# darkAlert/sports-field-homography

Hardware: AMD Instinct MI355X
Metric: frames/sec at 640x360 batch=16 (1/2/4/8 GPU) + homography L1 vs ref (higher is better)
Workload: dtype f16x3->f32 (2-way fp16 split operands = 22 significand bits, 3 fp16 MFMA products, fp32 accumulate; end-to-end error at the level of an fp32 run, see DESIGN.md section 2); 1 GPU; predict(): UNet seg + ResNet34-STN + nearest warp, 640x360, batch 16/GPU, req_outputs=theta,warp_mask; global_batch=16, precision=f16x3, range_fallbacks=0, range_rescales=0, range_raises=0, parallelism=single GPU

## Files before the change

include/sfh_amd.h:

```cpp
#ifndef SFH_AMD_H
#define SFH_AMD_H

#include <stdint.h>

#ifdef __cplusplus
extern "C" {
#endif

#define SFH_OK 0
#define SFH_E_ARG (-1)
#define SFH_E_LAUNCH (-2)

#define SFH_TILE_8x32 0
#define SFH_TILE_16x16 1
#define SFH_TILE_32x8 2
#define SFH_TILE_8x16 3
#define SFH_TILE_16x8 4

#define SFH_FMT_F32 0
#define SFH_FMT_S3 1
#define SFH_FMT_H2 2
#define SFH_FMT_FH2 3
#define SFH_H2_ACT_EXP 2

// ... 36 lines not shown
  int32_t h2_exp_src, h2_exp_dst, h2_exp_res;
  uint32_t* h2_range;
  int32_t wg_couts;
  int32_t split_arith;
  int32_t ksplit;
  int64_t ksplit_stride;
  const float* acc_init;
  double* stats_partial;
  int32_t stats_rows;
  const float* bwd_z;
  const float* bwd_mi;
  const float* bwd_gamma;
  const float* bwd_beta;
  const float* up_wpacked;
  const float* up_scale;
} sfh_conv_desc;

const char* sfh_last_error(void);
int sfh_version(void);

int sfh_conv_fwd(const sfh_conv_desc* d, void* stream);

int sfh_conv_s3_fwd(const sfh_conv_desc* d, void* stream);
int64_t sfh_packed_s3_weight_bytes(int ksize, int c0, int c1, int cout_virtual);
int sfh_pack_s3_weights(const float* w, void* packed, int ksize, int c0, int c1, int cout_virtual,
                        int mode, int aux, void* stream);
int sfh_f32_to_s3(const float* src, void* dst, int64_t rows, int W, int cs, void* stream);
int sfh_s3_to_f32(const void* src, float* dst, int64_t rows, int W, int cs, void* stream);

int64_t sfh_packed_h2_weight_bytes(int ksize, int c0, int c1, int cout_virtual);
int sfh_pack_h2_weights(const float* w, void* packed, int ksize, int c0, int c1, int cout_virtual,
                        int mode, int aux, int wexp, void* stream);
int sfh_f32_to_h2(const float* src, void* dst, int64_t rows, int W, int cs, int act_exp, uint32_t* overflow,
                  uint32_t* range, void* stream);
int sfh_h2_to_f32(const void* src, float* dst, int64_t rows, int W, int cs, int act_exp, void* stream);

int sfh_conv_small_fwd(const sfh_conv_desc* d, void* stream);

int sfh_conv_upfused_fwd(const sfh_conv_desc* d, void* stream);

int sfh_conv3x3_c4_fwd(const sfh_conv_desc* d, void* stream);
int sfh_pack_c4_weights(const float* w, float* packed, int cin, int cout, void* stream);

int sfh_frame_to_h2(const float* src_nchw, float* dst_nhwc4, void* dst_fh2, int batch, int C, int H, int W, int act_exp,
                    uint32_t* overflow, uint32_t* range, void* stream);
int64_t sfh_packed_c4h2_weight_bytes(int cout);
// ... 203 lines not shown
```

sports-field-homography_amd/_lib.py:

```python
import ctypes as C
import os

_HERE = os.path.dirname(os.path.abspath(__file__))
LIB_PATH = os.environ.get("SFH_AMD_LIB") or os.path.join(_HERE, "libsfh_amd.so")

TILE_8x32, TILE_16x16, TILE_32x8, TILE_8x16, TILE_16x8 = 0, 1, 2, 3, 4
OUT_NHWC, OUT_UPSCATTER2 = 0, 1
FMT_F32, FMT_S3, FMT_H2, FMT_FH2 = 0, 1, 2, 3
H2_ACT_EXP = 2
H2_LIMIT_BITS = 0x477FE000

_p = C.c_void_p
_i = C.c_int32


class ConvDesc(C.Structure):
    _fields_ = [
        ("src0", _p), ("c0", _i), ("cs0", _i), ("h0", _i), ("w0", _i), ("pool0", _i),
        ("src1", _p), ("c1", _i), ("cs1", _i), ("h1", _i), ("w1", _i), ("pad_top1", _i), ("pad_left1", _i),
        ("batch", _i), ("H", _i), ("W", _i), ("ksize", _i), ("stride", _i), ("tile", _i),
        ("wpacked", _p), ("scale", _p), ("shift", _p), ("cout", _i), ("relu", _i),
        ("residual", _p),
        ("dst", _p), ("dst_cs", _i), ("out_mode", _i),
        ("src_fmt", _i), ("dst_fmt", _i), ("dst_pool", _p), ("pool_cs", _i),
        ("residual_f32", _i), ("shift_border", _p), ("up_dst_h", _i), ("up_dst_w", _i),
        ("reverse_tiles", _i),
        ("head_w", _p), ("head_b", _p), ("head_nc", _i), ("head_skip_dst", _i),
        ("head_logits", _p), ("head_stn", _p), ("head_frame", _p),
        ("h2_overflow", _p), ("h2_exp_src", _i), ("h2_exp_dst", _i), ("h2_exp_res", _i), ("h2_range", _p),
        ("wg_couts", _i), ("split_arith", _i), ("ksplit", _i), ("ksplit_stride", C.c_int64), ("acc_init", _p),
        ("stats_partial", _p), ("stats_rows", _i),
        ("bwd_z", _p), ("bwd_mi", _p), ("bwd_gamma", _p), ("bwd_beta", _p),
        ("up_wpacked", _p), ("up_scale", _p),
    ]

    def __init__(self, *args, **kw):
        super().__init__(*args, **kw)
        if "h2_exp_src" not in kw:
            self.h2_exp_src = self.h2_exp_dst = self.h2_exp_res = H2_ACT_EXP


SIGNATURES = {
    "sfh_last_error": (C.c_char_p, []),
    "sfh_version": (C.c_int, []),
    "sfh_conv_fwd": (C.c_int, [C.POINTER(ConvDesc), _p]),
    "sfh_conv_s3_fwd": (C.c_int, [C.POINTER(ConvDesc), _p]),
    "sfh_packed_s3_weight_bytes": (C.c_int64, [C.c_int, C.c_int, C.c_int, C.c_int]),
    "sfh_pack_s3_weights": (C.c_int, [_p, _p, C.c_int, C.c_int, C.c_int, C.c_int, C.c_int, C.c_int, _p]),
    "sfh_f32_to_s3": (C.c_int, [_p, _p, C.c_int64, C.c_int, C.c_int, _p]),
    "sfh_s3_to_f32": (C.c_int, [_p, _p, C.c_int64, C.c_int, C.c_int, _p]),
    "sfh_packed_h2_weight_bytes": (C.c_int64, [C.c_int, C.c_int, C.c_int, C.c_int]),
    "sfh_pack_h2_weights": (C.c_int, [_p, _p, C.c_int, C.c_int, C.c_int, C.c_int, C.c_int, C.c_int, C.c_int, _p]),
    "sfh_f32_to_h2": (C.c_int, [_p, _p, C.c_int64, C.c_int, C.c_int, C.c_int, _p, _p, _p]),
    "sfh_h2_to_f32": (C.c_int, [_p, _p, C.c_int64, C.c_int, C.c_int, C.c_int, _p]),
    "sfh_conv3x3_c4_fwd": (C.c_int, [C.POINTER(ConvDesc), _p]),
    "sfh_pack_c4_weights": (C.c_int, [_p, _p, C.c_int, C.c_int, _p]),
    "sfh_frame_to_h2": (C.c_int, [_p, _p, _p, C.c_int, C.c_int, C.c_int, C.c_int, C.c_int, _p, _p, _p]),
    "sfh_packed_c4h2_weight_bytes": (C.c_int64, [C.c_int]),
    "sfh_pack_c4h2_weights": (C.c_int, [_p, _p, C.c_int, C.c_int, C.c_int, _p]),
    "sfh_conv3x3_c4h2_fwd": (C.c_int, [C.POINTER(ConvDesc), _p]),
    "sfh_conv_small_fwd": (C.c_int, [C.POINTER(ConvDesc), _p]),
    "sfh_conv_upfused_fwd": (C.c_int, [C.POINTER(ConvDesc), _p]),
    "sfh_packed_weight_floats": (C.c_int64, [C.c_int, C.c_int, C.c_int, C.c_int]),
    "sfh_pack_conv_weights": (C.c_int, [_p, _p, C.c_int, C.c_int, C.c_int, C.c_int, C.c_int, C.c_int, _p]),
    "sfh_space_to_depth2": (C.c_int, [_p, _p, C.c_int, C.c_int, C.c_int, C.c_int, _p]),
    "sfh_fold_bn": (C.c_int, [_p, _p, _p, _p, _p, C.c_float, C.c_int, C.c_int, _p, _p, _p]),
    "sfh_u8hwc_to_f32nchw": (C.c_int, [_p, _p, C.c_int, C.c_int, C.c_int, C.c_int, _p]),
    "sfh_u8hwc_area2_to_f32nchw": (C.c_int, [_p, _p, C.c_int, C.c_int, C.c_int, C.c_int, _p]),
    "sfh_u8hwc_areak_to_f32nchw": (C.c_int, [_p, _p, C.c_int, C.c_int, C.c_int, C.c_int, C.c_int, _p]),
# ... 120 lines not shown
```

sports-field-homography_amd/csrc/conv_s3.hip:

```cpp
#include <stdlib.h>

#include <type_traits>

#include "common.h"
#include "conv_epilogue.h"

typedef unsigned int u32x4 __attribute__((ext_vector_type(4)));
typedef unsigned int u32x2 __attribute__((ext_vector_type(2)));
typedef __bf16 bf16x8 __attribute__((ext_vector_type(8)));
typedef _Float16 f16x8 __attribute__((ext_vector_type(8)));

namespace {

constexpr unsigned kOOB = 0xFFFFFFF0u;

#ifndef SFH_STAGE_PRIO
#define SFH_STAGE_PRIO 0
#endif

template <int KS_, int STRIDE_, int SH_, int SW_, int TH_, int TW_, int NP_ = 3, int NWN_ = 2, int NWM_ = 2, bool STATS_ = false>
struct S3Cfg {
  static constexpr int KS = KS_, STRIDE = STRIDE_, NP = NP_, NWN = NWN_, NWM = NWM_;
  static constexpr bool STATS = STATS_;
  static constexpr int NT = 64 * NWM * NWN;
// ... 124 lines not shown
    }
  }
}

}

namespace {

#ifndef SFH_H2_WD
#define SFH_H2_WD 2
#endif
#ifndef SFH_H2_XD
#define SFH_H2_XD 2
#endif
#ifndef SFH_W128_NWM
#define SFH_W128_NWM 1
#endif
#ifndef SFH_W8_MIN_BLOCKS
#define SFH_W8_MIN_BLOCKS 384
#endif
#ifndef SFH_H2_WAVES_PER_SIMD
#define SFH_H2_WAVES_PER_SIMD 2
#endif
template <class C, bool DB>
__global__ __launch_bounds__(C::NT, (C::NP == 2 && !DB) ? SFH_H2_WAVES_PER_SIMD : 2) void conv_s3_kernel(const sfh_conv_desc d,
                                                                                                     const S3Geom g) {
  extern __shared__ __attribute__((aligned(16))) float smem_f[];
  u32x4* const lds = reinterpret_cast<u32x4*>(smem_f);
  typedef __attribute__((address_space(3))) void* lds_ptr_t;
  SFH_STAMP_INIT();
  SFH_CLOCK_BEGIN();

  const int tid = threadIdx.x;
  const int lane = tid & 63;
  const int wv = __builtin_amdgcn_readfirstlane(tid >> 6);
  const int wm = wv / C::NWN, wn = wv % C::NWN;
  const int lq = lane & 15, lg = lane >> 4;

  const int ksn = d.ksplit > 1 ? d.ksplit : 1;
  const int per_split = (int)(gridDim.x / (unsigned)ksn);
  const int ks = ksn > 1 ? (int)blockIdx.x / per_split : 0;
  const int bid = (int)blockIdx.x - ks * per_split;
  const int xcd = bid & 7, kk_ = bid >> 3;
  const int tpx = (g.ntiles + 7) >> 3;
  const int per = tpx * g.nb_group;
  const int gi = kk_ / per, rr = kk_ - gi * per;
  const int nb = gi * g.nb_group + rr % g.nb_group;
  const int tl = d.reverse_tiles ? tpx - 1 - rr / g.nb_group : rr / g.nb_group;
  const int tile = xcd * tpx + tl;
// ... 5 lines not shown
    r0 = ty * C::TH;
  } else {
    const int img = ty / g.tiles_y;
    r0 = (img << 16) | ((ty - img * g.tiles_y) * C::TH);
  }
  const int n0 = nb * C::NCO;

  const int nst0 = d.c0 / C::CKS;
  const int nst1 = d.src1 ? d.c1 / C::CKS : 0;
  const int nst = nst0 + nst1;
  const int st0 = ks * nst / ksn, st1 = (ks + 1) * nst / ksn;

  const __amdgpu_buffer_rsrc_t rs0 =
      __builtin_amdgcn_make_buffer_rsrc(const_cast<float*>(d.src0), 0, (int)g.bytes0, 0x00020000);
  const __amdgpu_buffer_rsrc_t rs1 = __builtin_amdgcn_make_buffer_rsrc(
      const_cast<float*>(d.src1 ? d.src1 : d.src0), 0, (int)(d.src1 ? g.bytes1 : 0u), 0x00020000);
  constexpr int NP = C::NP;
  constexpr unsigned WTAP = (unsigned)NP * 4u * 1024u;
  const unsigned wtotal = (unsigned)nst * C::NTAP * WTAP;
  const __amdgpu_buffer_rsrc_t rsw = __builtin_amdgcn_make_buffer_rsrc(
      const_cast<char*>(reinterpret_cast<const char*>(d.wpacked)) + (size_t)(nb * (C::NWN / 2) + (wn >> 1)) * wtotal, 0,
      (int)wtotal, 0x00020000);
  const unsigned wvoff = lane * 16u + (unsigned)(2 * (wn & 1)) * 1024u;

  int pad_y = C::PAD, pad_x = C::PAD;
  if (C::KS == 2) {
    const int qd = n0 / (d.cout >> 2);
    pad_y = 1 - (qd >> 1);
    pad_x = 1 - (qd & 1);
  }
  unsigned hoff[C::NSL];
  s3_halo_offsets<C>(d, g, 0, tid, r0, x0, pad_y, pad_x, hoff);

  auto dma_piece = [&](int st, int b, int i) {
    u32x4* const hb = lds + b * C::BUF;
    const bool first = st < nst0;
    constexpr unsigned SB = 64u * (unsigned)NP;
    const unsigned cb = first ? (unsigned)st * (SB * (unsigned)d.w0) : (unsigned)(st - nst0) * (SB * (unsigned)d.w1);
    __builtin_amdgcn_raw_ptr_buffer_load_lds(first ? rs0 : rs1, (lds_ptr_t)(hb + wv * 64 + C::NT * i), 16,
                                             (int)hoff[i], (int)cb, 0, 0);
  };
  auto dma_stage = [&](int st, int b) {
#pragma unroll
    for (int i = 0; i < C::NSL; ++i) dma_piece(st, b, i);
  };

  auto load_w = [&](u32x4 (&w)[NP][2], unsigned soff) {
#pragma unroll
    for (int p = 0; p < NP; ++p)
#pragma unroll
      for (int ni = 0; ni < 2; ++ni)
        w[p][ni] = __builtin_amdgcn_raw_buffer_load_b128(rsw, (int)(wvoff + ni * 1024u), (int)(soff + p * 4096u), 0);
  };

  const int pixbase0 = lg * C::HPIXP +
                       ((wm * C::MT_M / C::SUBX) * C::SH + lq / C::SW) * C::STRIDE * C::HW +
                       (lq % C::SW) * C::STRIDE;
  static_assert(C::MT_M % C::SUBX == 0, "a wave's pixel groups must start on a tile-row boundary");

  f32x4 acc[2][C::MT_M];
#pragma unroll
  for (int ni = 0; ni < 2; ++ni)
#pragma unroll
    for (int mi = 0; mi < C::MT_M; ++mi) acc[ni][mi] = (f32x4){0.f, 0.f, 0.f, 0.f};
  if constexpr (C::KS == 3 && C::STRIDE == 1) {
    if (d.acc_init) {
      const __amdgpu_buffer_rsrc_t ri =
          __builtin_amdgcn_make_buffer_rsrc(const_cast<float*>(d.acc_init), 0, (int)kOOB, 0x00020000);
      const unsigned cs_i = (unsigned)d.cout;
      const unsigned c_lane_i = (unsigned)(n0 + 32 * wn + 4 * lg);
#pragma unroll
      for (int mi = 0; mi < C::MT_M; ++mi) {
        const int sgi = wm * C::MT_M + mi;
        const int sy = sgi / C::SUBX, sx = sgi - sy * C::SUBX;
        const int oy = sy * C::SH + lq / C::SW, ox = sx * C::SW + lq % C::SW;
        const int x = x0 + ox, r = r0 + oy;
        const int b = (int)__umulhi((unsigned)r, g.rows_magic);
        const int y = r - b * g.rows_per_img;
        const bool ok = x < g.Wo && r < g.rows_total && y < g.Ho;
        const unsigned off = ok ? (((unsigned)(b * g.Ho + y) * (unsigned)g.Wo + (unsigned)x) * cs_i + c_lane_i) * 4u : kOOB;
#pragma unroll
        for (int ni = 0; ni < 2; ++ni)
          acc[ni][mi] = __builtin_bit_cast(f32x4, __builtin_amdgcn_raw_buffer_load_b128(ri, (int)off, ni * 64, 0));
      }
    }
  }

// ... 11 lines not shown
  auto stage = [&](int st, int cur, auto r0_tag) {
    constexpr int R0 = decltype(r0_tag)::value;
    constexpr int NSTEP = C::NTAP * C::MT_M;
    const u32x4* const halo = lds + cur * C::BUF;
    u32x4 xq[XD + 1][NP];
    auto ld_x = [&](int s, int buf) {
      const int t = s / C::MT_M, mi = s % C::MT_M;
      const int toff = (t / C::KS) * C::HW + (t % C::KS);
      const int moff = (mi / C::SUBX) * C::SH * C::STRIDE * C::HW + (mi % C::SUBX) * C::SW * C::STRIDE;
#pragma unroll
      for (int p = 0; p < NP; ++p) xq[buf][p] = halo[pixbase0 + (p * 4 * C::HPIXP + moff + toff)];
    };
#pragma unroll
    for (int i = 0; i < XD; ++i)
      if (i < NSTEP) ld_x(i, i);
    const int stn = st + 1 < st1 ? st + 1 : st;
#pragma unroll
    for (int s = 0; s < NSTEP; ++s) {
      const int t = s / C::MT_M, mi = s % C::MT_M;
      const int xb = s % (XD + 1);
      u32x4 (&wc)[NP][2] = wr[(R0 + t) % WD];
      u32x4 (&wnx)[NP][2] = wr[(R0 + t + WD - 1) % WD];
      if (s + XD < NSTEP) ld_x(s + XD, (s + XD) % (XD + 1));
      if (mi == 0) {
        load_w(wnx, wsoff);
        wsoff = (wsoff + WTAP <= wlast) ? wsoff + WTAP : wlast;
      }
      constexpr int PPS = C::NT == 512 ? C::NSL : (C::NSL + NSTEP - 1) / NSTEP;
      if (DB) {
#pragma unroll
        for (int q = 0; q < PPS; ++q)
          if (s * PPS + q < C::NSL) dma_piece(stn, cur ^ 1, s * PPS + q);
      }
      constexpr int NPROD = NP == 3 ? 6 : 3;
      constexpr int PW[6] = {0, 1, NP == 3 ? 2 : 0, 0, 1, 0}, PX[6] = {NP == 3 ? 2 : 1, NP == 3 ? 1 : 0, 0, 1, 0, 0};
#pragma unroll
      for (int k6 = 0; k6 < NPROD; ++k6)
#pragma unroll
        for (int ni = 0; ni < 2; ++ni) {
          if constexpr (NP == 3)
            acc[ni][mi] = __builtin_amdgcn_mfma_f32_16x16x32_bf16(as_bf(wc[PW[k6]][ni]), as_bf(xq[xb][PX[k6]]),
                                                                 acc[ni][mi], 0, 0, 0);
          else
            acc[ni][mi] = __builtin_amdgcn_mfma_f32_16x16x32_f16(as_hf(wc[PW[k6]][ni]), as_hf(xq[xb][PX[k6]]),
                                                                acc[ni][mi], 0, 0, 0);
        }
      __builtin_amdgcn_sched_group_barrier(0x008, 1, 0);
      __builtin_amdgcn_sched_group_barrier(0x100, NP, 0);
      __builtin_amdgcn_sched_group_barrier(0x008, 2 * NPROD - 1, 0);
      __builtin_amdgcn_sched_barrier(0);
    }
  };
  constexpr int SWAPS = C::NTAP % WD;
  static_assert((2 * C::NTAP) % WD == 0, "the stage loop is unrolled by two");

  dma_stage(st0, 0);
  if (SFH_STAGE_PRIO) __builtin_amdgcn_s_setprio(SFH_STAGE_PRIO);
  auto maybe_switch = [&](int st) {
    if (d.src1 && st + 1 == nst0) {
      s3_halo_offsets<C>(d, g, 1, tid, r0, x0, pad_y, pad_x, hoff);
    }
  };
  auto stage_barrier = [&]() {
    asm volatile("s_waitcnt vmcnt(0)" ::: "memory");
    __syncthreads();
  };
  if (DB) {
    for (int st = st0; st < st1; st += 2) {
      maybe_switch(st);
      stage_barrier();
      stage(st, 0, std::integral_constant<int, 0>{});
      if (st + 1 < st1) {
// ... 16 lines not shown
        }
        __syncthreads();
        dma_stage(st + 1, 0);
        SFH_STAMP(3);
        stage_barrier();
        SFH_STAMP(1);
        stage(st + 1, 0, std::integral_constant<int, SWAPS>{});
        SFH_STAMP(2);
      }
      if (st + 2 < st1) {
        if (d.src1 && st + 2 == nst0) {
          s3_halo_offsets<C>(d, g, 1, tid, r0, x0, pad_y, pad_x, hoff);
        }
        __syncthreads();
        dma_stage(st + 2, 0);
        SFH_STAMP(3);
      }
    }
  }
  if (SFH_STAGE_PRIO) __builtin_amdgcn_s_setprio(0);
  sfh_conv_epilogue<C, 2, C::MT_M, (NP == 3 ? 1 : 2)>(d, g, acc, n0 + 32 * wn, wm * C::MT_M, r0, x0, lq, lg,
                                                      (size_t)ks * (size_t)d.ksplit_stride,
                                                      (unsigned)(tile * C::NWM + wm));
  if (!DB) {
    SFH_STAMP(4);
    SFH_CLOCK_END();
    SFH_STAMP_FLUSH_AT(8);
  }

  if constexpr (C::KS == 3 && C::STRIDE == 1 && C::NWN == 2) {
    if (d.head_w) {
      float* const hl = smem_f;
      const int nc = d.head_nc;
      __syncthreads();
      for (int k = 0; k < nc; ++k) {
        f32x4 wk[2];
#pragma unroll
        for (int ni = 0; ni < 2; ++ni) wk[ni] = *reinterpret_cast<const f32x4*>(d.head_w + k * 64 + 32 * wn + ni * 16 + 4 * lg);
#pragma unroll
        for (int mi = 0; mi < C::MT_M; ++mi) {
          float p = 0.f;
#pragma unroll
          for (int ni = 0; ni < 2; ++ni)
#pragma unroll
            for (int j = 0; j < 4; ++j) p += acc[ni][mi][j] * wk[ni][j];
          p += __shfl_xor(p, 16);
// ... 9 lines not shown
        const int x = x0 + ox, r = r0 + oy;
        const int b = (int)__umulhi((unsigned)r, g.rows_magic);
        const int y = r - b * g.rows_per_img;
        if (x < g.Wo && r < g.rows_total && y < g.Ho) {
          float lgt[8];
#pragma unroll
          for (int k = 0; k < 8; ++k)
            lgt[k] = k < nc ? hl[(s * 16 + q) * 8 + k] + hl[((C::NSUBT + s) * 16 + q) * 8 + k] + d.head_b[k] : 0.f;
          const long hw = (long)g.Ho * g.Wo, pix = (long)y * g.Wo + x;
          for (int k = 0; k < nc; ++k) d.head_logits[((long)b * nc + k) * hw + pix] = lgt[k];
          if (d.head_stn) {
            const f32x4 fr = *reinterpret_cast<const f32x4*>(d.head_frame + ((long)b * hw + pix) * 4);
            float v8[8] = {0.f, 0.f, 0.f, 0.f, 0.f, 0.f, 0.f, 0.f};
            for (int k = 0; k < nc; ++k) v8[k] = lgt[k];
            for (int k = 0; k < 3 && nc + k < 8; ++k) v8[nc + k] = fr[k];
            float* o = d.head_stn + ((long)b * hw + pix) * 8;
            *reinterpret_cast<f32x4*>(o) = (f32x4){v8[0], v8[1], v8[2], v8[3]};
            *reinterpret_cast<f32x4*>(o + 4) = (f32x4){v8[4], v8[5], v8[6], v8[7]};
          }
        }
      }
    }
  }
}

template <int NP>
__global__ void pack_s3_weights_kernel(const float* __restrict__ w, unsigned short* __restrict__ packed,
                                       int ks, int c0, int c1, int coutv, int transposed, int aux, long total,
                                       float wscale) {
  const long idx = (long)blockIdx.x * blockDim.x + threadIdx.x;
  if (idx >= total) return;
  const int ntap = ks * ks;
  const int nst0 = c0 / 32, nst1 = c1 / 32, nst = nst0 + nst1;
  long r = idx;
  const int lane = r & 63; r >>= 6;
  const int ng = r & 3; r >>= 2;
  const int tap = r % ntap; r /= ntap;
  const int st = r % nst;
  const int nb = r / nst;
  const int ky = tap / ks, kx = tap % ks;
  const int cv = nb * 64 + ng * 16 + (lane & 15);
  const int cin_total = c0 + c1;
  const long base = ((((long)nb * nst + st) * ntap + tap) * NP) * 4096 + (long)ng * 1024 + lane * 16;
#pragma unroll
  for (int j = 0; j < 8; ++j) {
    const int cl = (st < nst0 ? st : st - nst0) * 32 + 8 * (lane >> 4) + j;
// ... 322 lines not shown
      unsigned short* dst = reinterpret_cast<unsigned short*>(dstv);
      u16x8 p0, p1, p2;
#pragma unroll
      for (int j = 0; j < 8; ++j) {
        const __bf16 v0 = (__bf16)v[j];
        const float r1 = v[j] - (float)v0;
        const __bf16 v1 = (__bf16)r1;
        const __bf16 v2 = (__bf16)(r1 - (float)v1);
        p0[j] = __builtin_bit_cast(unsigned short, v0);
        p1[j] = __builtin_bit_cast(unsigned short, v1);
        p2[j] = __builtin_bit_cast(unsigned short, v2);
      }
      const long e = s3_elem(row, x, c0, 0, W, cs);
      const long ps = 4L * W * 8;
      *reinterpret_cast<u16x8*>(dst + e) = p0;
      *reinterpret_cast<u16x8*>(dst + e + ps) = p1;
      *reinterpret_cast<u16x8*>(dst + e + 2 * ps) = p2;
    }
  }
  if constexpr (DFMT == SFH_FMT_H2) sfh_h2_report(over, overflow, range);
}

template <class C, bool DB>
int launch_s3(const sfh_conv_desc& d, hipStream_t stream) {
  S3Geom g;
  g.Ho = (d.H + C::PAD + C::PADA - C::KS) / C::STRIDE + 1;
  g.Wo = (d.W + C::PAD + C::PADA - C::KS) / C::STRIDE + 1;
  g.tiles_x = sfh_cdiv(g.Wo, C::TW);
  if (C::FLATROWS) {
    int zr = C::PAD;
    if ((g.Ho + zr) & 1) ++zr;
    if (zr == 0) zr = (g.Ho & 1) ? 1 : 0;
    g.rows_per_img = g.Ho + zr;
    g.rows_total = d.batch * g.rows_per_img;
    g.rows_magic = (unsigned)((1ULL << 32) / (unsigned)g.rows_per_img) + 1u;
    SFH_REQUIRE((unsigned long long)(g.rows_total + 64) * g.rows_per_img < (1ULL << 32),
                "conv_s3: flattened row space too large");
    g.tiles_y = sfh_cdiv(g.rows_total, C::TH);
    g.ntiles = g.tiles_x * g.tiles_y;
  } else {
    g.rows_total = 0;
    g.rows_per_img = g.Ho;
    g.rows_magic = 0;
    g.tiles_y = sfh_cdiv(g.Ho, C::TH);
    g.ntiles = g.tiles_x * g.tiles_y * d.batch;
    SFH_REQUIRE(g.Ho < 65536 && d.batch < 32768, "conv_s3: geometry too large");
  }
  const unsigned long long b0 = 2ULL * C::NP * d.batch * d.h0 * d.w0 * d.cs0;
  const unsigned long long b1 = d.src1 ? 2ULL * C::NP * d.batch * d.h1 * d.w1 * d.cs1 : 0ULL;
  SFH_REQUIRE(b0 < kOOB && b1 < kOOB, "conv_s3: a source tensor of %llu bytes exceeds the 4 GiB descriptor range; split the batch",
              b0 > b1 ? b0 : b1);
  g.bytes0 = (unsigned)b0;
  g.bytes1 = (unsigned)b1;
  g.nblk_n = d.cout / C::NCO;
  {
    const long wblock = (long)((d.c0 + (d.src1 ? d.c1 : 0)) / 32) * C::NTAP * (C::NP * 4096);
    const long budget = 64L << 20;
    int G = d.out_mode == SFH_OUT_UPSCATTER2 ? g.nblk_n : (int)(budget / (wblock > 0 ? wblock : 1));
    if (G < 1) G = 1;
    if (G > g.nblk_n) G = g.nblk_n;
    while (g.nblk_n % G) --G;
    g.nb_group = G;
  }
  const int ksn = d.ksplit > 1 ? d.ksplit : 1;
  const long nblocks = (long)sfh_cdiv(g.ntiles, 8) * 8 * g.nblk_n * ksn;
  SFH_REQUIRE(nblocks < (1L << 31), "conv_s3: grid too large");
  if constexpr (!DB && C::LDS_BYTES <= 160 * 1024) {
    if (nblocks <= 320) return launch_s3<C, true>(d, stream);
#ifdef SFH_KS2_DB
    if (C::KS == 2 && C::NWN == 2 && C::NP == 2) return launch_s3<C, true>(d, stream);
#endif
  }
  sfh_allow_big_lds(reinterpret_cast<const void*>(&conv_s3_kernel<C, DB>));
  hipLaunchKernelGGL((conv_s3_kernel<C, DB>), dim3((unsigned)nblocks), dim3(C::NT),
                     DB ? C::LDS_BYTES : C::LDS_BYTES / 2, stream, d, g);
  return sfh_check_launch("conv_s3_kernel");
}

}

extern "C" int64_t sfh_packed_s3_weight_bytes(int ksize, int c0, int c1, int cout_virtual) {
  if ((ksize != 1 && ksize != 2 && ksize != 3 && ksize != 4) || c0 <= 0 || c0 % 32 || c1 < 0 || c1 % 32 || cout_virtual <= 0 ||
      cout_virtual % 64)
    return -1;
  return (int64_t)(cout_virtual / 64) * ((c0 + c1) / 32) * (ksize * ksize) * 3 * 4096;
}

extern "C" int sfh_pack_s3_weights(const float* w, void* packed, int ksize, int c0, int c1, int cout_virtual,
                                   int mode, int aux, void* stream) {
  const int64_t n = sfh_packed_s3_weight_bytes(ksize, c0, c1, cout_virtual);
  SFH_REQUIRE(n > 0, "pack_s3_weights: bad geometry ks=%d c0=%d c1=%d cout=%d", ksize, c0, c1, cout_virtual);
  SFH_REQUIRE(w && packed, "pack_s3_weights: null pointer");
  SFH_REQUIRE((mode == 0 && ksize != 4) || (mode == 1 && ksize == 1 && c1 == 0 && cout_virtual % 256 == 0) ||
                  (mode == 2 && ksize == 4 && c1 == 0 && aux > 0 && aux <= c0 / 4) ||
                  (mode == 3 && c1 == 0 && (ksize == 1 || ksize == 3) && aux > 0 && aux <= cout_virtual) ||
// ... 114 lines not shown
                                 const void* residual, int res_fmt, int exp_res, int relu, int64_t rows, int W, int C,
                                 void* dst, int dst_fmt, int exp_dst, uint32_t* overflow, uint32_t* range, void* stream) {
  SFH_REQUIRE(slabs && shift && dst && nslabs >= 1 && nslabs <= 64 && rows > 0 && W > 0 && C > 0 && C % 32 == 0,
              "splitk_finish: bad arguments (nslabs=%d, C=%d must be a multiple of 32)", nslabs, C);
  SFH_REQUIRE(slab_stride % 16 == 0 && slab_stride >= rows * W * C * 4, "splitk_finish: slab_stride=%lld is smaller than a slab",
              (long long)slab_stride);
  SFH_REQUIRE(dst_fmt == SFH_FMT_F32 || dst_fmt == SFH_FMT_S3 || dst_fmt == SFH_FMT_H2, "splitk_finish: dst_fmt=%d", dst_fmt);
  SFH_REQUIRE(!residual || res_fmt == SFH_FMT_F32 || res_fmt == SFH_FMT_S3 || res_fmt == SFH_FMT_H2, "splitk_finish: res_fmt=%d", res_fmt);
  SFH_REQUIRE(exp_dst >= -64 && exp_dst <= 64 && exp_res >= -64 && exp_res <= 64, "splitk_finish: exponent out of range");
  const int xchunks = (W + 15) / 16;
  const long total = rows * (C / 32) * xchunks * 64;
  const dim3 grid((unsigned)((total + 255) / 256));
#define SFH_FINISH(F_)                                                                                               \
  hipLaunchKernelGGL(splitk_finish_kernel<F_>, grid, dim3(256), 0, (hipStream_t)stream, slabs, nslabs,               \
                     (long)(slab_stride / 4), shift, residual, res_fmt, ldexpf(1.f, -exp_res), relu, W, C, xchunks, \
                     total, dst, ldexpf(1.f, exp_dst), overflow, range)
  if (dst_fmt == SFH_FMT_H2) SFH_FINISH(SFH_FMT_H2);
  else if (dst_fmt == SFH_FMT_S3) SFH_FINISH(SFH_FMT_S3);
  else SFH_FINISH(SFH_FMT_F32);
#undef SFH_FINISH
  return sfh_check_launch("splitk_finish_kernel");
}

extern "C" int sfh_conv_s3_fwd(const sfh_conv_desc* dp, void* stream_) {
  SFH_REQUIRE(dp, "conv_s3_fwd: null descriptor");
  const sfh_conv_desc& d = *dp;
  hipStream_t stream = (hipStream_t)stream_;
  SFH_REQUIRE(d.src0 && d.wpacked && d.scale && d.shift && d.dst, "conv_s3_fwd: null pointer");
  SFH_REQUIRE(d.src_fmt == SFH_FMT_S3 || d.src_fmt == SFH_FMT_H2, "conv_s3_fwd: sources must be S3 or H2 tensors (src_fmt=%d)", d.src_fmt);
  SFH_REQUIRE(d.dst_fmt == SFH_FMT_F32 || d.dst_fmt == d.src_fmt,
              "conv_s3_fwd: the destination is fp32 or the sources' own split format (src_fmt=%d, dst_fmt=%d)", d.src_fmt, d.dst_fmt);
  SFH_REQUIRE(d.batch > 0 && d.H > 0 && d.W > 0, "conv_s3_fwd: empty geometry");
  SFH_REQUIRE(d.h2_exp_dst >= -64 && d.h2_exp_dst <= 64 && d.h2_exp_res >= -64 && d.h2_exp_res <= 64,
              "conv_s3_fwd: h2_exp_dst=%d / h2_exp_res=%d out of range (-64 .. 64)", d.h2_exp_dst, d.h2_exp_res);
  SFH_REQUIRE(d.cout > 0 && d.cout % 64 == 0, "conv_s3_fwd: cout=%d must be a multiple of 64", d.cout);
  SFH_REQUIRE(d.c0 > 0 && d.c0 % 32 == 0 && d.cs0 >= d.c0, "conv_s3_fwd: c0=%d must be a multiple of 32 (cs0=%d)", d.c0, d.cs0);
  SFH_REQUIRE(!d.pool0, "conv_s3_fwd: pool-on-load is not available for S3 sources (use the producer's dst_pool)");
  SFH_REQUIRE((d.h0 == d.H && d.w0 == d.W) ||
                  (d.ksize == 2 && (d.H == d.h0 || d.H == d.h0 + 1) && (d.W == d.w0 || d.W == d.w0 + 1)),
              "conv_s3_fwd: source 0 is %dx%d, frame is %dx%d", d.h0, d.w0, d.H, d.W);
  SFH_REQUIRE((!d.up_dst_h && !d.up_dst_w) || d.ksize == 2, "conv_s3_fwd: up_dst_h/w exist only for the 2x2 up-scatter conv");
  if (d.ksize == 2)
    SFH_REQUIRE((d.up_dst_h == 0 || (d.up_dst_h >= 2 * d.h0 && d.up_dst_h <= 2 * d.H)) &&
                    (d.up_dst_w == 0 || (d.up_dst_w >= 2 * d.w0 && d.up_dst_w <= 2 * d.W)),
                "conv_s3_fwd: up_dst %dx%d does not match the source %dx%d", d.up_dst_h, d.up_dst_w, d.h0, d.w0);
  SFH_REQUIRE(d.stride == 1 || (d.stride == 2 && !d.src1 && !d.dst_pool && d.out_mode == SFH_OUT_NHWC),
              "conv_s3_fwd: stride 2 supports a single source, plain output");
// ... 61 lines not shown
    }                                                                                                         \
  }
  SFH_S3CASE_W8(3, 1, SFH_TILE_8x32, 1, 16, 8, 32)
  SFH_S3CASE_W8(3, 1, SFH_TILE_16x16, 1, 16, 16, 16)
  SFH_S3CASE_W8(3, 1, SFH_TILE_32x8, 2, 8, 32, 8)
  SFH_S3CASE_W8(2, 1, SFH_TILE_8x32, 1, 16, 8, 32)
  SFH_S3CASE_W8(2, 1, SFH_TILE_16x16, 1, 16, 16, 16)
  if (SFH_W128_NWM == 2) {
    SFH_S3CASE_W8(2, 1, SFH_TILE_32x8, 2, 8, 32, 8)
  }
#undef SFH_S3CASE_W8
  if (w8h_ok && d.wg_couts == 128 && !d.stats_partial) {
    if (d.tile == SFH_TILE_8x16) return launch_s3<S3Cfg<3, 1, 1, 16, 8, 16, 2, 4, 1>, true>(d, stream);
    if (d.tile == SFH_TILE_16x8) return launch_s3<S3Cfg<3, 1, 2, 8, 16, 8, 2, 4, 1>, true>(d, stream);
  }
#define SFH_S3CASE(KS, ST, TILE, SH, SW, TH, TW)                      \
  if (d.ksize == KS && d.stride == ST && d.tile == TILE) {             \
    if (d.src_fmt == SFH_FMT_H2) {                                     \
      using CFG = S3Cfg<KS, ST, SH, SW, TH, TW, 2>;                    \
      if constexpr ((KS == 3 || KS == 1) && ST == 1) {                 \
        using CFGS = S3Cfg<KS, ST, SH, SW, TH, TW, 2, 2, 2, true>;     \
        if (d.stats_partial) return launch_s3<CFGS, false>(d, stream); \
      }                                                                \
      return launch_s3<CFG, false>(d, stream);                         \
    }                                                                  \
    using CFG = S3Cfg<KS, ST, SH, SW, TH, TW, 3>;                      \
    return launch_s3<CFG, false>(d, stream);                           \
  }
  SFH_S3CASE(3, 1, SFH_TILE_8x32, 1, 16, 8, 32)
  SFH_S3CASE(3, 1, SFH_TILE_16x16, 1, 16, 16, 16)
  SFH_S3CASE(3, 1, SFH_TILE_32x8, 2, 8, 32, 8)
  SFH_S3CASE(1, 1, SFH_TILE_8x32, 1, 16, 8, 32)
  SFH_S3CASE(1, 1, SFH_TILE_16x16, 1, 16, 16, 16)
  SFH_S3CASE(1, 1, SFH_TILE_32x8, 2, 8, 32, 8)
  SFH_S3CASE(2, 1, SFH_TILE_8x32, 1, 16, 8, 32)
  SFH_S3CASE(2, 1, SFH_TILE_16x16, 1, 16, 16, 16)
  SFH_S3CASE(2, 1, SFH_TILE_32x8, 2, 8, 32, 8)
  SFH_S3CASE(3, 1, SFH_TILE_8x16, 1, 16, 8, 16)
  SFH_S3CASE(3, 1, SFH_TILE_16x8, 2, 8, 16, 8)
  SFH_S3CASE(4, 1, SFH_TILE_8x32, 1, 16, 8, 32)
  SFH_S3CASE(4, 1, SFH_TILE_16x16, 1, 16, 16, 16)
  SFH_S3CASE(4, 1, SFH_TILE_32x8, 2, 8, 32, 8)
  SFH_S3CASE(3, 2, SFH_TILE_8x16, 1, 16, 8, 16)
  SFH_S3CASE(3, 2, SFH_TILE_16x8, 2, 8, 16, 8)
  SFH_S3CASE(1, 2, SFH_TILE_8x16, 1, 16, 8, 16)
  SFH_S3CASE(1, 2, SFH_TILE_16x8, 2, 8, 16, 8)
#undef SFH_S3CASE
  sfh_set_error("conv_s3_fwd: unsupported ksize=%d stride=%d tile=%d", d.ksize, d.stride, d.tile);
  return SFH_E_ARG;
}
```

sports-field-homography_amd/engine.py:

```python
import ctypes
import math
import os
import threading

import torch

from . import _lib
from ._lib import ConvDesc

BN_EPS = 1e-5

_TILES = ((_lib.TILE_8x32, 8, 32), (_lib.TILE_16x16, 16, 16), (_lib.TILE_32x8, 32, 8))


_STREAM_TLS = threading.local()


def _stream():
    stack = getattr(_STREAM_TLS, "stack", None)
    if stack:
        return stack[-1]
    return ctypes.c_void_p(torch.cuda.current_stream().cuda_stream)


# ... 628 lines not shown
            n = lib.sfh_packed_weight_floats(ksize, c0, 0, self.cout)
            if n <= 0:
                raise ValueError(f"unsupported backward-data geometry ksize={ksize} c0={c0} cout={self.cout}")
            self.wpacked = torch.empty(n, dtype=torch.float32, device=dev)
            _lib.check(lib.sfh_pack_conv_weights(_ptr(w), _ptr(self.wpacked), ksize, c0, 0, self.cout, mode, aux,
                                                 _stream()), "pack_conv_weights")
        self.scale, self.shift = _unit_epilogue(self.cout, dev, self.escale)
        self._shared_scale = True
        return self

    def _fold_exp_src(self, e):
        if e == self.exp_src:
            return
        if self._shared_scale:
            raise ValueError("this layer's epilogue scale is shared with other layers: its source exponent is fixed")
        f = 2.0 ** (self.exp_src - e)
        vec_op(self.scale, factor=f, out=self.scale)
        self.escale *= f
        self.exp_src = e

    def run(self, src0, batch, H, W, dst, src1=None, pool0=False, pad1=(0, 0), residual=None, tile=None,
            dst_pool=None, up_dst=None, head=None, wg_couts=0, exp_src=None, exp_dst=None, exp_res=None,
            range_word=None, ksplit=0, slabs=None, acc_init=None, scale=None, shift_border=None, stats=None, bwd=None,
            small=None):
        lib = _lib.load()
        d = ConvDesc()
        if (self.fmt == "h2" or getattr(self, "c4h2", False)) and exp_src is not None:
            self._fold_exp_src(int(exp_src))
        d.h2_exp_src = self.exp_src
        if exp_dst is not None:
            d.h2_exp_dst = int(exp_dst)
        if exp_res is not None:
            d.h2_exp_res = int(exp_res)
        d.src0 = src0.data_ptr()
        d.c0, d.cs0 = self.c0, _chan(src0)
        d.h0, d.w0 = _hw(src0)
        if _fmt_of(src0) != self.fmt or (src1 is not None and _fmt_of(src1) != self.fmt):
            raise ValueError(f"layer of format {self.fmt} got a source of dtype {src0.dtype}")
        d.src_fmt = _fmt_code(src0)
        d.dst_fmt = _fmt_code(dst)
        if self.fmt is not None and _fmt_of(dst) not in (None, self.fmt):
            raise ValueError(f"layer of format {self.fmt} cannot write a {dst.dtype} destination")
        for t in (dst_pool, residual):
            if t is not None and _fmt_of(t) not in (None, _fmt_of(dst)):
                raise ValueError(f"dst_pool / residual of dtype {t.dtype} beside a {dst.dtype} destination")
        ovf = getattr(self, "overflow", None)
        d.h2_overflow = ovf.data_ptr() if (ovf is not None and _fmt_of(dst) == "h2") else None
# ... 103 lines not shown
        small_ok = (self.fmt == "h2" and self.ksize == 3 and self.stride == 1 and not self.transposed and src1 is None
                    and dst_pool is None and head is None and acc_init is None and stats is None and not (ksplit and ksplit > 1)
                    and not d.residual_f32 and sb is None and not self.c4)
        if small and not small_ok:
            raise ValueError("the small-map kernel takes a plain 3x3 stride-1 H2 conv (one source, no pooled output / head / "
                             "acc_init / statistics / split-K)")
        if small is None and small_ok and _SMALL_MAP and wg_couts == 0 and tile is None:
            small = choose_small_map(batch, ho, wo, zr, self.cout, d.tile)
        if small:
            fwd = lib.sfh_conv_small_fwd
            d.wg_couts = _SMALL_MAP_BUFFERS + (16 if _SMALL_MAP_WS_ORDER else 0)
        if self.c4:
            if src0.shape[-1] != 4 or pool0 or dst_pool is not None:
                raise ValueError("the <=4-channel first-layer kernel needs an fp32 NHWC source with 4 stored channels")
            fwd = lib.sfh_conv3x3_c4h2_fwd if self.c4h2 else lib.sfh_conv3x3_c4_fwd
            if self.c4h2:
                d.src_fmt = _lib.FMT_FH2
        tm = PackedConv.timer
        if tm is not None and not tm.wants(self.tag):
            tm = None
        if tm is not None:
            e0, e1 = torch.cuda.Event(enable_timing=True), torch.cuda.Event(enable_timing=True)
            e0.record()
        _lib.check(fwd(ctypes.byref(d), _stream()), "conv_s3_fwd" if self.s3 else "conv_fwd")
        if finish is not None:
            finish()
        if tm is not None:
            e1.record()
            kk = 49 if self.ksize == 4 else (4 if self.transposed else self.ksize * self.ksize)
            cin = self.stem_cin if self.ksize == 4 else self.c0 + self.c1
            flops = 2.0 * batch * ho * wo * self.cout_real * kk * cin
            fpp = getattr(self, "flops_per_out_pixel", None)
            executed = None
            if fpp is not None:
                executed = 2.0 * batch * ho * wo * self.cout * 4 * self.c0
                flops = fpp * batch * (2 * ho) * (2 * wo)
            bpe = {"h2": 4, "s3": 6}.get(self.fmt, 4)
            nbytes = batch * d.h0 * d.w0 * self.c0 * bpe + self.wpacked.numel() * self.wpacked.element_size()
            if src1 is not None:
                nbytes += batch * d.h1 * d.w1 * self.c1 * bpe
            obpe = {"h2": 4, "s3": 6}.get(_fmt_of(dst), 4)
            if not (head is not None and head.get("skip_dst")):
                nbytes += exp[0] * exp[1] * exp[2] * self.cout_real * (4 if (ksplit and ksplit > 1) else obpe)
            if dst_pool is not None:
                nbytes += batch * (ho // 2) * (wo // 2) * self.cout_real * obpe
            if head is not None:
                nbytes += batch * ho * wo * head["nc"] * 4
            for t in (residual, acc_init):
                if t is not None:
                    nbytes += t.numel() * t.element_size()
            tm.records.append((self.tag, flops, e0, e1, executed, float(nbytes)))
        return dst


# ... 379 lines not shown
        if tm is not None:
            e0, e1 = torch.cuda.Event(enable_timing=True), torch.cuda.Event(enable_timing=True)
            e0.record()
        _lib.check(lib.sfh_stem7x7_fwd(ctypes.byref(d), _stream()), "stem7x7_fwd")
        if tm is not None:
            e1.record()
            tm.records.append((self.tag, 2.0 * B * ho * wo * 64 * 49 * self.cin, e0, e1))
        return dst


class ResNetEngine:

    def __init__(self, rn, in_channels, device, precision="bf16x6", overflow=None, ranges=None):
        if precision not in PRECISIONS:
            raise ValueError(f"precision={precision!r}: expected one of {sorted(PRECISIONS)}")
        self.fmt = fmt = PRECISIONS[precision]
        self.s3 = fmt is not None
        s3 = self.s3
        self.overflow = overflow if fmt == "h2" else None
        self.ranges = (ranges if ranges is not None else H2Ranges(device)) if fmt == "h2" else _NoRanges()
        self.steps = []
        self._last_out = None
        self.splitk = os.environ.get("SFH_SPLITK", "1") != "0"
        self.device = device
        self.ws = _Workspace(device)
        self.cin = in_channels
        self.cs_in = -(-in_channels // 4) * 4
        if (4 * self.cs_in) % 16:
            self.cs_in = -(-in_channels // 8) * 8
        L = {}
        wx = {}
        if fmt == "h2":
            ws_ = [p.detach() for p in rn.parameters() if p.dim() == 4 and p.is_contiguous()]
            for w, (mx, _) in zip(ws_, absminmax(ws_)):
                wx[w.data_ptr()] = h2_weight_exp(mx)
        def PC(w, *a, **k):
            return PackedConv(w, *a, wexp=wx.get(w.data_ptr()), **k)
        L["stem"] = PC(rn.conv0.weight, None, rn.bn1, 4, 4 * self.cs_in, stem_cin=in_channels, tag="resnet")
        self.stem7 = (StemConv(rn.conv0, rn.bn1, in_channels, fmt=fmt, overflow=self.overflow, wexp=wx.get(rn.conv0.weight.data_ptr()))
                      if (s3 and self.cs_in == 8 and rn.conv0.out_channels == 64
                                                                  and os.environ.get("SFH_STEM7", "1") != "0") else None)
        self.blocks = []
        for li in range(1, 5):
            for bi, blk in enumerate(getattr(rn, f"layer{li}")):
                name = f"layer{li}.{bi}"
                cin = blk.conv1.in_channels
# ... 61 lines not shown
            do((), lambda s2d=s2d: L["stem"].run(s2d, B, H2, W2, c1))
        h, w = (H2 - 1) // 2 + 1, (W2 - 1) // 2 + 1

        def act(name, hh, ww, c):
            if s3:
                rg.register("rn." + name)
                return ws.get(name, split_shape(fmt, B, hh, ww, c), _SPLIT[fmt][0]), "rn." + name
            return ws.get(name, (B, hh, ww, c)), None

        nx = None
        if s3:
            x, nx = act("pool.s3", h, w, 64)
            ovf = self.overflow
            do((nx,), lambda x=x, nx=nx: _lib.check(lib.sfh_maxpool3x3s2_split_fwd(
                _ptr(c1), _ptr(x), B, H2, W2, 64, _SPLIT[fmt][2], rg.exp(nx),
                ctypes.c_void_p(ovf.data_ptr()) if (ovf is not None and fmt == "h2") else None,
                ctypes.c_void_p(rg.word_ptr(nx)) if rg.word_ptr(nx) else None, _stream()), "maxpool3x3s2_split"))
        else:
            x = ws.get("pool", (B, h, w, 64))
            do((), lambda x=x: _lib.check(lib.sfh_maxpool3x3s2_fwd(_ptr(c1), _ptr(x), B, H2, W2, 64, _stream()), "maxpool3x3s2"))
        for name, width, cout, stride, has_down, bottleneck in self.blocks:
            ho, wo = (h - 1) // stride + 1, (w - 1) // stride + 1

            def conv(layer, src, nsrc, hh, ww, dst, ndst, residual=None, nres=None):
                pc = L[layer]
                ks, slabs = 1, None
                if s3 and use_splitk:
                    oh, ow = (hh - 1) // pc.stride + 1, (ww - 1) // pc.stride + 1
                    ks = choose_ksplit(B, oh, ow, pc.stride, pc.cout, (pc.c0 + pc.c1) // 32, pc.ksize)
                    if ks > 1:
                        slabs = ws.get(f"slabs{ks}x{oh}x{ow}x{pc.cout}", (ks, B, oh, ow, pc.cout))
                do((ndst,) if ndst else (), lambda: pc.run(src, B, hh, ww, dst, residual=residual, ksplit=ks, slabs=slabs,
                                                           **rg.args(nsrc, ndst, nres)))
            if has_down:
                idn, nidn = act(name + ".idn", ho, wo, cout)
                conv(name + ".down", x, nx, h, w, idn, nidn)
            else:
                idn, nidn = x, nx
            out, nout = act(name + ".out", ho, wo, cout)
            if bottleneck:
                t1, nt1 = act(name + ".t1", h, w, width)
                conv(name + ".conv1", x, nx, h, w, t1, nt1)
                t2, nt2 = act(name + ".t2", ho, wo, width)
                conv(name + ".conv2", t1, nt1, h, w, t2, nt2)
                conv(name + ".conv3", t2, nt2, ho, wo, out, nout, residual=idn, nres=nidn)
            else:
                t, nt = act(name + ".t", ho, wo, width)
                conv(name + ".conv1", x, nx, h, w, t, nt)
                conv(name + ".conv2", t, nt, ho, wo, out, nout, residual=idn, nres=nidn)
            x, nx, h, w = out, nout, ho, wo
        if s3:
            xf = ws.get("final.f32", (B, h, w, _chan(x)))
            do((), lambda x=x, nx=nx, xf=xf: _split_to_f32_into(x, xf, rg.exp(nx)))
            x = xf
        theta = torch.empty((B, 9), dtype=torch.float32, device=x.device)
        pooled = ws.get("pooled", (B, x.shape[3]))
        do((), lambda x=x, h=h, w=w: _lib.check(
            lib.sfh_avgpool_linear_fwd(_ptr(x), _ptr(self.reg_w), _ptr(self.reg_b), B, h, w, x.shape[3], 9,
                                       _ptr(pooled), _ptr(theta), _stream()), "avgpool_linear"))
        self._last_out = theta.view(B, 1, 3, 3)
        return self._last_out


# ... 231 lines not shown
```

Before: 1251 frames/s.

## Fuse ResNet downsample 1x1 projection into the 3x3 stride-2 conv1 kernel

```diff
diff --git a/include/sfh_amd.h b/include/sfh_amd.h
--- a/include/sfh_amd.h
+++ b/include/sfh_amd.h
@@ -82,6 +82,7 @@
 int sfh_conv_fwd(const sfh_conv_desc* d, void* stream);
 
 int sfh_conv_s3_fwd(const sfh_conv_desc* d, void* stream);
+int sfh_conv_s3_down_fwd(const sfh_conv_desc* d, const sfh_conv_desc* down, void* stream);
 int64_t sfh_packed_s3_weight_bytes(int ksize, int c0, int c1, int cout_virtual);
 int sfh_pack_s3_weights(const float* w, void* packed, int ksize, int c0, int c1, int cout_virtual,
                         int mode, int aux, void* stream);
diff --git a/sports-field-homography_amd/_lib.py b/sports-field-homography_amd/_lib.py
--- a/sports-field-homography_amd/_lib.py
+++ b/sports-field-homography_amd/_lib.py
@@ -45,6 +45,7 @@
     "sfh_version": (C.c_int, []),
     "sfh_conv_fwd": (C.c_int, [C.POINTER(ConvDesc), _p]),
     "sfh_conv_s3_fwd": (C.c_int, [C.POINTER(ConvDesc), _p]),
+    "sfh_conv_s3_down_fwd": (C.c_int, [C.POINTER(ConvDesc), C.POINTER(ConvDesc), _p]),
     "sfh_packed_s3_weight_bytes": (C.c_int64, [C.c_int, C.c_int, C.c_int, C.c_int]),
     "sfh_pack_s3_weights": (C.c_int, [_p, _p, C.c_int, C.c_int, C.c_int, C.c_int, C.c_int, C.c_int, _p]),
     "sfh_f32_to_s3": (C.c_int, [_p, _p, C.c_int64, C.c_int, C.c_int, _p]),
diff --git a/sports-field-homography_amd/csrc/conv_s3.hip b/sports-field-homography_amd/csrc/conv_s3.hip
--- a/sports-field-homography_amd/csrc/conv_s3.hip
+++ b/sports-field-homography_amd/csrc/conv_s3.hip
@@ -170,9 +170,9 @@
 #ifndef SFH_H2_WAVES_PER_SIMD
 #define SFH_H2_WAVES_PER_SIMD 2
 #endif
-template <class C, bool DB>
-__global__ __launch_bounds__(C::NT, (C::NP == 2 && !DB) ? SFH_H2_WAVES_PER_SIMD : 2) void conv_s3_kernel(const sfh_conv_desc d,
-                                                                                                     const S3Geom g) {
+template <class C, bool DB, bool DOWN>
+__device__ __forceinline__ void conv_s3_body(const sfh_conv_desc& d, const S3Geom& g, const sfh_conv_desc& dd) {
+  static_assert(!DOWN || (C::KS == 3 && C::STRIDE == 2), "the fused projection rides on a 3x3 stride-2 conv");
   extern __shared__ __attribute__((aligned(16))) float smem_f[];
   u32x4* const lds = reinterpret_cast<u32x4*>(smem_f);
   typedef __attribute__((address_space(3))) void* lds_ptr_t;
@@ -224,6 +224,10 @@
       const_cast<char*>(reinterpret_cast<const char*>(d.wpacked)) + (size_t)(nb * (C::NWN / 2) + (wn >> 1)) * wtotal, 0,
       (int)wtotal, 0x00020000);
   const unsigned wvoff = lane * 16u + (unsigned)(2 * (wn & 1)) * 1024u;
+  const unsigned wtotal_d = (unsigned)nst * WTAP;
+  const __amdgpu_buffer_rsrc_t rswd = __builtin_amdgcn_make_buffer_rsrc(
+      const_cast<char*>(reinterpret_cast<const char*>(dd.wpacked)) + (size_t)(nb * (C::NWN / 2) + (wn >> 1)) * wtotal_d, 0,
+      (int)wtotal_d, 0x00020000);
 
   int pad_y = C::PAD, pad_x = C::PAD;
   if (C::KS == 2) {
@@ -265,6 +269,12 @@
   for (int ni = 0; ni < 2; ++ni)
 #pragma unroll
     for (int mi = 0; mi < C::MT_M; ++mi) acc[ni][mi] = (f32x4){0.f, 0.f, 0.f, 0.f};
+  f32x4 accd[2][DOWN ? C::MT_M : 1];
+  u32x4 wd[C::NP][2];
+#pragma unroll
+  for (int ni = 0; ni < 2; ++ni)
+#pragma unroll
+    for (int mi = 0; mi < (DOWN ? C::MT_M : 1); ++mi) accd[ni][mi] = (f32x4){0.f, 0.f, 0.f, 0.f};
   if constexpr (C::KS == 3 && C::STRIDE == 1) {
     if (d.acc_init) {
       const __amdgpu_buffer_rsrc_t ri =
@@ -322,6 +332,15 @@
       u32x4 (&wc)[NP][2] = wr[(R0 + t) % WD];
       u32x4 (&wnx)[NP][2] = wr[(R0 + t + WD - 1) % WD];
       if (s + XD < NSTEP) ld_x(s + XD, (s + XD) % (XD + 1));
+      if constexpr (DOWN) {
+        if (s == 0) {
+#pragma unroll
+          for (int p = 0; p < NP; ++p)
+#pragma unroll
+            for (int ni = 0; ni < 2; ++ni)
+              wd[p][ni] = __builtin_amdgcn_raw_buffer_load_b128(rswd, (int)(wvoff + ni * 1024u), (int)((unsigned)st * WTAP + p * 4096u), 0);
+        }
+      }
       if (mi == 0) {
         load_w(wnx, wsoff);
         wsoff = (wsoff + WTAP <= wlast) ? wsoff + WTAP : wlast;
@@ -345,9 +364,26 @@
             acc[ni][mi] = __builtin_amdgcn_mfma_f32_16x16x32_f16(as_hf(wc[PW[k6]][ni]), as_hf(xq[xb][PX[k6]]),
                                                                 acc[ni][mi], 0, 0, 0);
         }
+      constexpr int CT = C::NTAP / 2;
+      if constexpr (DOWN) {
+        if (t == CT) {
+#pragma unroll
+          for (int k6 = 0; k6 < NPROD; ++k6)
+#pragma unroll
+            for (int ni = 0; ni < 2; ++ni) {
+              if constexpr (NP == 3)
+                accd[ni][mi] = __builtin_amdgcn_mfma_f32_16x16x32_bf16(as_bf(wd[PW[k6]][ni]), as_bf(xq[xb][PX[k6]]),
+                                                                       accd[ni][mi], 0, 0, 0);
+              else
+                accd[ni][mi] = __builtin_amdgcn_mfma_f32_16x16x32_f16(as_hf(wd[PW[k6]][ni]), as_hf(xq[xb][PX[k6]]),
+                                                                      accd[ni][mi], 0, 0, 0);
+            }
+        }
+      }
       __builtin_amdgcn_sched_group_barrier(0x008, 1, 0);
       __builtin_amdgcn_sched_group_barrier(0x100, NP, 0);
       __builtin_amdgcn_sched_group_barrier(0x008, 2 * NPROD - 1, 0);
+      if (DOWN && t == CT) __builtin_amdgcn_sched_group_barrier(0x008, 2 * NPROD, 0);
       __builtin_amdgcn_sched_barrier(0);
     }
   };
@@ -410,6 +446,8 @@
   sfh_conv_epilogue<C, 2, C::MT_M, (NP == 3 ? 1 : 2)>(d, g, acc, n0 + 32 * wn, wm * C::MT_M, r0, x0, lq, lg,
                                                       (size_t)ks * (size_t)d.ksplit_stride,
                                                       (unsigned)(tile * C::NWM + wm));
+  if constexpr (DOWN)
+    sfh_conv_epilogue<C, 2, C::MT_M, (NP == 3 ? 1 : 2)>(dd, g, accd, n0 + 32 * wn, wm * C::MT_M, r0, x0, lq, lg);
   if (!DB) {
     SFH_STAMP(4);
     SFH_CLOCK_END();
@@ -465,6 +503,18 @@
       }
     }
   }
+}
+
+template <class C, bool DB>
+__global__ __launch_bounds__(C::NT, (C::NP == 2 && !DB) ? SFH_H2_WAVES_PER_SIMD : 2) void conv_s3_kernel(const sfh_conv_desc d,
+                                                                                                     const S3Geom g) {
+  conv_s3_body<C, DB, false>(d, g, d);
+}
+
+template <class C, bool DB>
+__global__ __launch_bounds__(C::NT, (C::NP == 2 && !DB) ? SFH_H2_WAVES_PER_SIMD : 2) void conv_s3_down_kernel(
+    const sfh_conv_desc d, const S3Geom g, const sfh_conv_desc dd) {
+  conv_s3_body<C, DB, true>(d, g, dd);
 }
 
 template <int NP>
@@ -833,7 +883,7 @@
 }
 
 template <class C, bool DB>
-int launch_s3(const sfh_conv_desc& d, hipStream_t stream) {
+int launch_s3(const sfh_conv_desc& d, hipStream_t stream, const sfh_conv_desc* dd = nullptr) {
   S3Geom g;
   g.Ho = (d.H + C::PAD + C::PADA - C::KS) / C::STRIDE + 1;
   g.Wo = (d.W + C::PAD + C::PADA - C::KS) / C::STRIDE + 1;
@@ -877,11 +927,20 @@
   const long nblocks = (long)sfh_cdiv(g.ntiles, 8) * 8 * g.nblk_n * ksn;
   SFH_REQUIRE(nblocks < (1L << 31), "conv_s3: grid too large");
   if constexpr (!DB && C::LDS_BYTES <= 160 * 1024) {
-    if (nblocks <= 320) return launch_s3<C, true>(d, stream);
+    if (nblocks <= 320) return launch_s3<C, true>(d, stream, dd);
 #ifdef SFH_KS2_DB
     if (C::KS == 2 && C::NWN == 2 && C::NP == 2) return launch_s3<C, true>(d, stream);
 #endif
   }
+  if constexpr (C::KS == 3 && C::STRIDE == 2) {
+    if (dd) {
+      sfh_allow_big_lds(reinterpret_cast<const void*>(&conv_s3_down_kernel<C, DB>));
+      hipLaunchKernelGGL((conv_s3_down_kernel<C, DB>), dim3((unsigned)nblocks), dim3(C::NT),
+                         DB ? C::LDS_BYTES : C::LDS_BYTES / 2, stream, d, g, *dd);
+      return sfh_check_launch("conv_s3_down_kernel");
+    }
+  }
+  SFH_REQUIRE(!dd, "conv_s3: the fused projection needs a 3x3 stride-2 launch");
   sfh_allow_big_lds(reinterpret_cast<const void*>(&conv_s3_kernel<C, DB>));
   hipLaunchKernelGGL((conv_s3_kernel<C, DB>), dim3((unsigned)nblocks), dim3(C::NT),
                      DB ? C::LDS_BYTES : C::LDS_BYTES / 2, stream, d, g);
@@ -1042,7 +1101,7 @@
   return sfh_check_launch("splitk_finish_kernel");
 }
 
-extern "C" int sfh_conv_s3_fwd(const sfh_conv_desc* dp, void* stream_) {
+static int conv_s3_fwd_impl(const sfh_conv_desc* dp, void* stream_, const sfh_conv_desc* dd) {
   SFH_REQUIRE(dp, "conv_s3_fwd: null descriptor");
   const sfh_conv_desc& d = *dp;
   hipStream_t stream = (hipStream_t)stream_;
@@ -1150,10 +1209,10 @@
         using CFGS = S3Cfg<KS, ST, SH, SW, TH, TW, 2, 2, 2, true>;     \
         if (d.stats_partial) return launch_s3<CFGS, false>(d, stream); \
       }                                                                \
-      return launch_s3<CFG, false>(d, stream);                         \
+      return launch_s3<CFG, false>(d, stream, dd);                     \
     }                                                                  \
     using CFG = S3Cfg<KS, ST, SH, SW, TH, TW, 3>;                      \
-    return launch_s3<CFG, false>(d, stream);                           \
+    return launch_s3<CFG, false>(d, stream, dd);                       \
   }
   SFH_S3CASE(3, 1, SFH_TILE_8x32, 1, 16, 8, 32)
   SFH_S3CASE(3, 1, SFH_TILE_16x16, 1, 16, 16, 16)
@@ -1177,3 +1236,22 @@
   sfh_set_error("conv_s3_fwd: unsupported ksize=%d stride=%d tile=%d", d.ksize, d.stride, d.tile);
   return SFH_E_ARG;
 }
+
+extern "C" int sfh_conv_s3_fwd(const sfh_conv_desc* dp, void* stream) { return conv_s3_fwd_impl(dp, stream, nullptr); }
+
+extern "C" int sfh_conv_s3_down_fwd(const sfh_conv_desc* dp, const sfh_conv_desc* ddp, void* stream) {
+  SFH_REQUIRE(dp && ddp, "conv_s3_down_fwd: null descriptor");
+  const sfh_conv_desc& d = *dp;
+  const sfh_conv_desc& dd = *ddp;
+  SFH_REQUIRE(d.ksize == 3 && d.stride == 2 && !(d.ksplit > 1) && !d.stats_partial && !d.acc_init && !d.head_w && d.wg_couts == 0,
+              "conv_s3_down_fwd: the carrying launch must be a plain 3x3 stride-2 conv (no split-K / statistics / acc_init / head)");
+  SFH_REQUIRE(dd.wpacked && dd.scale && dd.shift && dd.dst, "conv_s3_down_fwd: null pointer in the projection's descriptor");
+  SFH_REQUIRE(dd.ksize == 1 && dd.stride == 2 && dd.src0 == d.src0 && !dd.src1 && dd.c0 == d.c0 && dd.cs0 == d.cs0 && dd.h0 == d.h0 &&
+                  dd.w0 == d.w0 && dd.batch == d.batch && dd.H == d.H && dd.W == d.W && dd.src_fmt == d.src_fmt && dd.cout == d.cout,
+              "conv_s3_down_fwd: the projection must be a 1x1 stride-2 conv over the same source with the same couts");
+  SFH_REQUIRE((dd.dst_fmt == SFH_FMT_F32 || dd.dst_fmt == dd.src_fmt) && dd.dst_cs >= dd.cout && dd.out_mode == SFH_OUT_NHWC &&
+                  !dd.residual && !dd.dst_pool && !dd.head_w && !dd.head_skip_dst && !(dd.ksplit > 1) && !dd.stats_partial &&
+                  !dd.acc_init && !dd.shift_border && !dd.up_dst_h && !dd.up_dst_w && dd.h2_exp_dst >= -64 && dd.h2_exp_dst <= 64,
+              "conv_s3_down_fwd: the projection writes a plain output (fp32 or the source format, no residual / pooled output / head)");
+  return conv_s3_fwd_impl(dp, stream, ddp);
+}
diff --git a/sports-field-homography_amd/engine.py b/sports-field-homography_amd/engine.py
--- a/sports-field-homography_amd/engine.py
+++ b/sports-field-homography_amd/engine.py
@@ -674,7 +674,7 @@
     def run(self, src0, batch, H, W, dst, src1=None, pool0=False, pad1=(0, 0), residual=None, tile=None,
             dst_pool=None, up_dst=None, head=None, wg_couts=0, exp_src=None, exp_dst=None, exp_res=None,
             range_word=None, ksplit=0, slabs=None, acc_init=None, scale=None, shift_border=None, stats=None, bwd=None,
-            small=None):
+            small=None, down=None):
         lib = _lib.load()
         d = ConvDesc()
         if (self.fmt == "h2" or getattr(self, "c4h2", False)) and exp_src is not None:
@@ -824,7 +824,27 @@
         if tm is not None:
             e0, e1 = torch.cuda.Event(enable_timing=True), torch.cuda.Event(enable_timing=True)
             e0.record()
-        _lib.check(fwd(ctypes.byref(d), _stream()), "conv_s3_fwd" if self.s3 else "conv_fwd")
+        if down is not None:
+            dl, ddst, dexp, drange = down
+            if (not self.s3 or self.ksize != 3 or self.stride != 2 or finish is not None or small or dl.ksize != 1
+                    or dl.stride != 2 or dl.fmt != self.fmt or dl.c0 != self.c0 or dl.cout != self.cout):
+                raise ValueError("down: a 3x3 stride-2 split-operand layer without split-K carries a 1x1 stride-2 layer")
+            if dl.fmt == "h2" and exp_src is not None:
+                dl._fold_exp_src(int(exp_src))
+            dd = ConvDesc.from_buffer_copy(d)
+            dd.ksize, dd.tile = 1, d.tile
+            dd.wpacked, dd.scale, dd.shift = dl.wpacked.data_ptr(), dl.scale.data_ptr(), dl.shift.data_ptr()
+            dd.relu, dd.residual, dd.residual_f32 = 1 if dl.relu else 0, None, 0
+            dd.dst, dd.dst_cs, dd.dst_fmt = ddst.data_ptr(), _chan(ddst), _fmt_code(ddst)
+            if (ddst.shape[0],) + _hw(ddst) != exp or _chan(ddst) < dl.cout_real:
+                raise ValueError(f"down dst shape {tuple(ddst.shape)} does not match {exp + (dl.cout_real,)}")
+            if dexp is not None:
+                dd.h2_exp_dst = int(dexp)
+            dd.h2_overflow = ovf.data_ptr() if (ovf is not None and _fmt_of(ddst) == "h2") else None
+            dd.h2_range = drange if (drange and _fmt_of(ddst) == "h2") else None
+            _lib.check(lib.sfh_conv_s3_down_fwd(ctypes.byref(d), ctypes.byref(dd), _stream()), "conv_s3_down_fwd")
+        else:
+            _lib.check(fwd(ctypes.byref(d), _stream()), "conv_s3_fwd" if self.s3 else "conv_fwd")
         if finish is not None:
             finish()
         if tm is not None:
@@ -832,6 +852,8 @@
             kk = 49 if self.ksize == 4 else (4 if self.transposed else self.ksize * self.ksize)
             cin = self.stem_cin if self.ksize == 4 else self.c0 + self.c1
             flops = 2.0 * batch * ho * wo * self.cout_real * kk * cin
+            if down is not None:
+                flops += 2.0 * batch * ho * wo * down[0].cout_real * cin
             fpp = getattr(self, "flops_per_out_pixel", None)
             executed = None
             if fpp is not None:
@@ -1257,6 +1279,7 @@
         self.steps = []
         self._last_out = None
         self.splitk = os.environ.get("SFH_SPLITK", "1") != "0"
+        self.fuse_down = True
         self.device = device
         self.ws = _Workspace(device)
         self.cin = in_channels
@@ -1364,23 +1387,37 @@
         for name, width, cout, stride, has_down, bottleneck in self.blocks:
             ho, wo = (h - 1) // stride + 1, (w - 1) // stride + 1
 
-            def conv(layer, src, nsrc, hh, ww, dst, ndst, residual=None, nres=None):
-                pc = L[layer]
+            def ksplit_of(pc, hh, ww):
                 ks, slabs = 1, None
                 if s3 and use_splitk:
                     oh, ow = (hh - 1) // pc.stride + 1, (ww - 1) // pc.stride + 1
                     ks = choose_ksplit(B, oh, ow, pc.stride, pc.cout, (pc.c0 + pc.c1) // 32, pc.ksize)
                     if ks > 1:
                         slabs = ws.get(f"slabs{ks}x{oh}x{ow}x{pc.cout}", (ks, B, oh, ow, pc.cout))
+                return ks, slabs
+
+            def conv(layer, src, nsrc, hh, ww, dst, ndst, residual=None, nres=None):
+                pc = L[layer]
+                ks, slabs = ksplit_of(pc, hh, ww)
                 do((ndst,) if ndst else (), lambda: pc.run(src, B, hh, ww, dst, residual=residual, ksplit=ks, slabs=slabs,
                                                            **rg.args(nsrc, ndst, nres)))
+            fused = (has_down and not bottleneck and s3 and self.fuse_down and stride == 2
+                     and ksplit_of(L[name + ".conv1"], h, w)[0] == 1)
             if has_down:
                 idn, nidn = act(name + ".idn", ho, wo, cout)
-                conv(name + ".down", x, nx, h, w, idn, nidn)
+                if not fused:
+                    conv(name + ".down", x, nx, h, w, idn, nidn)
             else:
                 idn, nidn = x, nx
             out, nout = act(name + ".out", ho, wo, cout)
-            if bottleneck:
+            if fused:
+                t, nt = act(name + ".t", ho, wo, width)
+                pc, pd = L[name + ".conv1"], L[name + ".down"]
+                do(tuple(n for n in (nt, nidn) if n),
+                   lambda pc=pc, pd=pd, x=x, nx=nx, h=h, w=w, t=t, nt=nt, idn=idn, nidn=nidn: pc.run(
+                       x, B, h, w, t, down=(pd, idn, rg.exp(nidn), rg.word_ptr(nidn)), **rg.args(nx, nt)))
+                conv(name + ".conv2", t, nt, ho, wo, out, nout, residual=idn, nres=nidn)
+            elif bottleneck:
                 t1, nt1 = act(name + ".t1", h, w, width)
                 conv(name + ".conv1", x, nx, h, w, t1, nt1)
                 t2, nt2 = act(name + ".t2", ho, wo, width)
```

Result: no change. 1250 frames/s, median of 4 (-0.0%).
